# colmap/glomap

Hardware: NVIDIA H100
Metric: observations/sec per BA LM-iteration (higher is better)
Workload: dtype f64

## Files before the change

glomap_b200/csrc/ba_kernels_ext.cuh:

```cuda
#pragma once
#include "ba_kernels_v3.cuh"

namespace b200 {

struct ExtView {
  int C, K, S;
  const IntrVarRec* ivar;
  const unsigned char* sensor_var;
};

template <bool WK, bool WS>
struct ObsFull {
  double Jr[6], Jt[6], Jp[6], r[2], rho0;
  double Jk[WK ? 2 : 1][kMaxBlockDof];
  double Jsr[WS ? 6 : 1], Jst[WS ? 6 : 1];
  bool valid;
};

template <bool WK, bool WS>
__device__ __forceinline__ void obs_full(const double4& q4, const double4& t4, const double* __restrict__ ir,
                                         const IntrVarRec& iv, const double* __restrict__ sr, bool svar, double X0,
                                         double X1, double X2, double2 xy, double huber_a, ObsFull<WK, WS>& o) {
  const int mask = (int)(__double_as_longlong(t4.w) & 0xff);
  const double q[4] = {q4.x, q4.y, q4.z, q4.w};
// ... 120 lines not shown
  const double4 q4c = ld_rec32(cam_rec + (size_t)cam * kCamRec);
  const double4 t4c = ld_rec32(cam_rec + (size_t)cam * kCamRec + 4);
  const int blk = v.seg_intr[warp];
  const double* irc = intr_rec + (size_t)blk * kIntrRec;
  const double* src = sensor_of_seg(v, warp);
  const int sidx = v.S > 0 ? v.seg_sensor[warp] : 0;
  const bool svar = v.S > 0 && ex.sensor_var && ex.sensor_var[sidx];
  IntrVarRec iv{};
  if (WHAT == 1) iv = ex.ivar[blk];
  int target = cam;
  if (WHAT == 1) {
    if (iv.mb == 0) return;
    target = ex.C + blk;
  }
  if (WHAT == 2) {
    if (!svar) return;
    target = ex.C + ex.K + sidx;
  }
  double U[21], g[6];
#pragma unroll
  for (int k = 0; k < 21; ++k) U[k] = 0.0;
#pragma unroll
  for (int k = 0; k < 6; ++k) g[k] = 0.0;
  for (int i = b + lane; i < e; i += 32) {
    const int pt = v.pt_c[i];
    const double2 xy = v.xy_c[i];
    const double X0 = points[3 * (size_t)pt], X1 = points[3 * (size_t)pt + 1], X2 = points[3 * (size_t)pt + 2];
    ObsFull<WHAT == 1, WHAT == 2> o;
    obs_full<WHAT == 1, WHAT == 2>(q4c, t4c, irc, iv, src, svar, X0, X1, X2, xy, huber_a, o);
    double Jb[2][6];
#pragma unroll
    for (int a = 0; a < 2; ++a)
#pragma unroll
      for (int k = 0; k < 3; ++k) {
        if (WHAT == 0) { Jb[a][k] = o.Jr[3 * a + k]; Jb[a][3 + k] = o.Jt[3 * a + k]; }
        if (WHAT == 2) { Jb[a][k] = o.Jsr[WHAT == 2 ? 3 * a + k : 0]; Jb[a][3 + k] = o.Jst[WHAT == 2 ? 3 * a + k : 0]; }
      }
    if (WHAT == 1) {
#pragma unroll
      for (int a = 0; a < 2; ++a) {
#pragma unroll
        for (int j = 0; j < kMaxBlockDof; ++j) Jb[a][j] = o.Jk[WHAT == 1 ? a : 0][j];
        Jb[a][5] = 0.0;
      }
    }
    int idx = 0;
#pragma unroll
    for (int i2 = 0; i2 < 6; ++i2) {
#pragma unroll
      for (int j = i2; j < 6; ++j) U[idx++] += Jb[0][i2] * Jb[0][j] + Jb[1][i2] * Jb[1][j];
      g[i2] += Jb[0][i2] * o.r[0] + Jb[1][i2] * o.r[1];
    }
  }
#pragma unroll
  for (int k = 0; k < 21; ++k) {
    const double s = warp_sum(U[k]);
    if (lane == k && s != 0.0) atomicAdd(&v.U[(size_t)target * 21 + k], s);
  }
#pragma unroll
  for (int k = 0; k < 6; ++k) {
    const double s = warp_sum(g[k]);
    if (lane == 21 + k && s != 0.0) atomicAdd(&v.gc[(size_t)target * 6 + k], s);
  }
}

template <int MODE, bool WK, bool WS>
__global__ void __launch_bounds__(kEllThreads) bax_pass_a(BAView v, EllView ell, ExtView ex, BAViewV2 v2,
                                                           const double* __restrict__ cam_rec,
                                                           const double* __restrict__ intr_rec,
                                                           const double* __restrict__ x, const double* __restrict__ points,
                                                           double* __restrict__ points_new, double huber_a, double radius,
                                                           double* __restrict__ bscal, const PcgCtl* __restrict__ ctl) {
  __shared__ double scratch[32];
  if (ctl && ctl->done) return;
  const int slot = blockIdx.x * kEllThreads + threadIdx.x;
  const int lane = threadIdx.x & 31;
  const int g = slot >> 5;
  double b0 = 0, b1 = 0, b2 = 0, b3 = 0;
  if (g < ell.n_groups) {
    const int pt = ell.pt[slot];
    const int mylen = ell.len[slot];
    const int r0 = ell.row0[g], nrow = ell.row0[g + 1] - r0;
    double X0 = 0, X1 = 0, X2 = 0;
    if (pt >= 0) {
      X0 = points[3 * (size_t)pt]; X1 = points[3 * (size_t)pt + 1]; X2 = points[3 * (size_t)pt + 2];
    }
    double s0 = 0, s1 = 0, s2 = 0;
    for (int j = 0; j < nrow; ++j) {
      if (j >= mylen) continue;
      const size_t idx = ((size_t)r0 + j) * 32 + lane;
      const int cam = ell.cam[idx];
      const double2 xy = ell.xy[idx];
      const double4 q4 = ld_rec32(cam_rec + (size_t)cam * kCamRec);
      const double4 t4 = ld_rec32(cam_rec + (size_t)cam * kCamRec + 4);
      const int sidx = ell.sensor ? (int)ell.sensor[idx] : 0;
      const double* sr = ell.sensor ? v.sensor_rec + (size_t)sidx * kSensorRec : nullptr;
      const int blk = obs_intr_idx(t4, sr);
      const double* ir = intr_rec + (size_t)blk * kIntrRec;
      const bool svar = WS && ell.sensor && ex.sensor_var && ex.sensor_var[sidx];
      IntrVarRec iv{};
      if (WK) iv = ex.ivar[blk];
      ObsFull<WK, WS> o;
      obs_full<WK, WS>(q4, t4, ir, iv, sr, svar, X0, X1, X2, xy, huber_a, o);
      double xc[6], xk[kMaxBlockDof], xs[6];
#pragma unroll
      for (int k = 0; k < 6; ++k) xc[k] = x[(size_t)cam * 6 + k];
#pragma unroll
      for (int k = 0; k < kMaxBlockDof; ++k) xk[k] = WK ? x[(size_t)(ex.C + blk) * 6 + k] : 0.0;
#pragma unroll
      for (int k = 0; k < 6; ++k) xs[k] = (WS && svar) ? x[(size_t)(ex.C + ex.K + sidx) * 6 + k] : 0.0;
      double t0, t1;
      obs_apply<WK, WS>(o, xc, xk, xs, t0, t1);
      s0 += o.Jp[0] * t0 + o.Jp[3] * t1;
      s1 += o.Jp[1] * t0 + o.Jp[4] * t1;
      s2 += o.Jp[2] * t0 + o.Jp[5] * t1;
    }
// ... 53 lines not shown
                                                 const double* __restrict__ x, double huber_a, double* __restrict__ y,
                                                 const PcgCtl* __restrict__ ctl) {
  if (ctl && ctl->done) return;
  const int warp = (blockIdx.x * blockDim.x + threadIdx.x) >> 5;
  const int lane = threadIdx.x & 31;
  if (warp >= v.n_segs) return;
  const int cam = v.seg_cam[warp];
  const int b = v.seg_begin[warp], e = v.seg_end[warp];
  const double4 q4c = ld_rec32(cam_rec + (size_t)cam * kCamRec);
  const double4 t4c = ld_rec32(cam_rec + (size_t)cam * kCamRec + 4);
  const int blk = v.seg_intr[warp];
  const double* irc = intr_rec + (size_t)blk * kIntrRec;
  const double* src = sensor_of_seg(v, warp);
  const int sidx = v.S > 0 ? v.seg_sensor[warp] : 0;
  const bool svar = WS && v.S > 0 && ex.sensor_var && ex.sensor_var[sidx];
  IntrVarRec iv{};
  if (WK) iv = ex.ivar[blk];
  double xc[6], xk[kMaxBlockDof], xs[6];
#pragma unroll
  for (int k = 0; k < 6; ++k) xc[k] = x ? x[(size_t)cam * 6 + k] : 0.0;
#pragma unroll
  for (int k = 0; k < kMaxBlockDof; ++k) xk[k] = (WK && x) ? x[(size_t)(ex.C + blk) * 6 + k] : 0.0;
#pragma unroll
  for (int k = 0; k < 6; ++k) xs[k] = (WS && svar && x) ? x[(size_t)(ex.C + ex.K + sidx) * 6 + k] : 0.0;
  double ac[6] = {0, 0, 0, 0, 0, 0}, ak[kMaxBlockDof] = {0, 0, 0, 0, 0}, as[6] = {0, 0, 0, 0, 0, 0};
  for (int i = b + lane; i < e; i += 32) {
    const int pt = v.pt_c[i];
    const double2 xy = v.xy_c[i];
    const double X0 = points[3 * (size_t)pt], X1 = points[3 * (size_t)pt + 1], X2 = points[3 * (size_t)pt + 2];
    const double4 z = *reinterpret_cast<const double4*>(v2.z4 + 4 * (size_t)pt);
    ObsFull<WK, WS> o;
    obs_full<WK, WS>(q4c, t4c, irc, iv, src, svar, X0, X1, X2, xy, huber_a, o);
    double t0, t1;
    obs_apply<WK, WS>(o, xc, xk, xs, t0, t1);
    t0 -= o.Jp[0] * z.x + o.Jp[1] * z.y + o.Jp[2] * z.z;
    t1 -= o.Jp[3] * z.x + o.Jp[4] * z.y + o.Jp[5] * z.z;
#pragma unroll
    for (int k = 0; k < 3; ++k) {
      ac[k] += o.Jr[k] * t0 + o.Jr[3 + k] * t1;
      ac[3 + k] += o.Jt[k] * t0 + o.Jt[3 + k] * t1;
    }
    if (WK) {
#pragma unroll
      for (int j = 0; j < kMaxBlockDof; ++j) ak[j] += o.Jk[0][j] * t0 + o.Jk[WK ? 1 : 0][j] * t1;
    }
    if (WS) {
#pragma unroll
      for (int k = 0; k < 3; ++k) {
        as[k] += o.Jsr[WS ? k : 0] * t0 + o.Jsr[WS ? 3 + k : 0] * t1;
        as[3 + k] += o.Jst[WS ? k : 0] * t0 + o.Jst[WS ? 3 + k : 0] * t1;
      }
    }
  }
#pragma unroll
  for (int k = 0; k < 6; ++k) {
    const double s = warp_sum(ac[k]);
    if (lane == k && s != 0.0) atomicAdd(&y[(size_t)cam * 6 + k], s);
  }
  if (WK) {
#pragma unroll
    for (int j = 0; j < kMaxBlockDof; ++j) {
      const double s = warp_sum(ak[j]);
      if (lane == 8 + j && j < iv.mb && s != 0.0) atomicAdd(&y[(size_t)(ex.C + blk) * 6 + j], s);
    }
  }
  if (WS) {
#pragma unroll
    for (int k = 0; k < 6; ++k) {
      const double s = warp_sum(as[k]);
      if (lane == 16 + k && svar && s != 0.0) atomicAdd(&y[(size_t)(ex.C + ex.K + sidx) * 6 + k], s);
    }
  }
}

__global__ void bax_update_extras(ExtView ex, const IntrVarRec* __restrict__ ivar, const int* __restrict__ intr_model,
                                  const double* __restrict__ intr, double* __restrict__ intr_new,
                                  const double* __restrict__ sq, const double* __restrict__ st, double* __restrict__ sq_new,
                                  double* __restrict__ st_new, const double* __restrict__ dc, const double* __restrict__ gc,
                                  const double* __restrict__ resid, const double* __restrict__ Dc,
                                  const double* __restrict__ jscale_c, const double* __restrict__ blk_used, int count_norms,
                                  double* __restrict__ cscal) {
  const int i = blockIdx.x * blockDim.x + threadIdx.x;
  double a0 = 0, a1 = 0, a2 = 0, a3 = 0, a4 = 0;
  if (i < ex.K) {
    const IntrVarRec iv = ivar[i];
    const size_t blk = (size_t)(ex.C + i);
    double p[12];
#pragma unroll
    for (int j = 0; j < 12; ++j) p[j] = intr[(size_t)i * 12 + j];
    for (int j = 0; j < iv.mb; ++j) {
      const size_t k = blk * 6 + j;
      if (!(jscale_c[k] >= 0.0)) continue;
      const double d = dc[k];
      a0 += gc[k] * d;
      a1 += resid[k] * d;
      a2 += Dc[k] * d * d;
      a3 += d * d;
      p[iv.pidx[j]] += d;
    }
    if (iv.mb > 0 && blk_used[blk] > 0.0) {
      const int npar = intr_model[i] == 0 ? 3 : (intr_model[i] == 3 ? 5 : 4);
      for (int j = 0; j < npar; ++j) a4 += intr[(size_t)i * 12 + j] * intr[(size_t)i * 12 + j];
    }
#pragma unroll
    for (int j = 0; j < 12; ++j) intr_new[(size_t)i * 12 + j] = p[j];
  } else if (i < ex.K + ex.S) {
    const int s = i - ex.K;
    const size_t blk = (size_t)(ex.C + ex.K + s);
    double d[6];
    bool rvar = false, tvar = false;
#pragma unroll
    for (int k = 0; k < 6; ++k) {
      const size_t j = blk * 6 + k;
      const bool var = jscale_c[j] >= 0.0;
      d[k] = var ? dc[j] : 0.0;
      if (var) {
        a0 += gc[j] * d[k];
        a1 += resid[j] * d[k];
        a2 += Dc[j] * d[k] * d[k];
        if (k < 3) rvar = true; else tvar = true;
      }
    }
    const bool in_problem = ex.sensor_var && ex.sensor_var[s] && blk_used[blk] > 0.0;
    const double q[4] = {sq[4 * s], sq[4 * s + 1], sq[4 * s + 2], sq[4 * s + 3]};
    double qn[4] = {q[0], q[1], q[2], q[3]};
// ... 43 lines not shown
```

glomap_b200/csrc/ba_kernels_v2.cuh:

```cuda
#pragma once
#include "ba_kernels.cuh"
#include "pcg.cuh"

namespace b200 {

struct BAViewV2 {
  const double* Ap;
  double* z4;
  const double* pts4;
  double* Ufk = nullptr;
  const IntrVarRec* ivar = nullptr;
  int C = 0;
};

template <int NK>
__device__ __forceinline__ void obs_intr_jac(const ObsCore& o, const Intr& in, const IntrVarRec& iv,
                                             double Jk[2][NK > 0 ? NK : 1]) {
#pragma unroll
  for (int j = 0; j < NK; ++j) {
    double jx = 0.0, jy = 0.0;
    if (j < iv.mb) intr_param_jac(in, iv.pidx[j], o.uv[0], o.uv[1], 1.0, jx, jy);
    if (!o.valid) jx = jy = 0.0;
    Jk[0][j] = jx;
    Jk[1][j] = jy;
  }
}
template <int NK>
__device__ __forceinline__ void obs_intr_rows(const ObsCore& o, const Intr& in, const IntrVarRec& iv,
                                              const double Jp[6], double Jk[2][NK > 0 ? NK : 1],
                                              double B[NK > 0 ? 3 * NK : 1]) {
  obs_intr_jac<NK>(o, in, iv, Jk);
#pragma unroll
  for (int j = 0; j < NK; ++j)
#pragma unroll
    for (int c = 0; c < 3; ++c) B[3 * j + c] = o.rho1 * (Jp[c] * Jk[0][j] + Jp[3 + c] * Jk[1][j]);
}

struct SegRec {
  double R[9];
  double4 t4;
  Intr in;
  const double* sr;
};
__device__ __forceinline__ void seg_records(const BAView& v, int seg, int cam, const double* __restrict__ cam_rec,
                                            const double* __restrict__ intr_rec, SegRec& s) {
  const double4 q4 = ld_rec32(cam_rec + (size_t)cam * kCamRec);
  s.t4 = ld_rec32(cam_rec + (size_t)cam * kCamRec + 4);
  s.in = ld_intr(intr_rec + (size_t)v.seg_intr[seg] * kIntrRec);
  s.sr = sensor_of_seg(v, seg);
  const double q[4] = {q4.x, q4.y, q4.z, q4.w};
  quat_to_R(q, s.R);
}
__device__ __forceinline__ void to_sensor(const double* __restrict__ sr, double x[3]) {
  if (!sr) return;
  const double x0 = x[0], x1 = x[1], x2 = x[2];
#pragma unroll
  for (int k = 0; k < 3; ++k) x[k] = sr[3 * k] * x0 + sr[3 * k + 1] * x1 + sr[3 * k + 2] * x2;
}
__device__ __forceinline__ void cam_frame_jac(const ObsCore& o, const double r[3], double a[2], double w[3]) {
  const ProjJac& p = o.pj;
  const double t0 = r[0] - p.u * r[2], t1 = r[1] - p.v * r[2];
  const double c = o.rho1 * p.iz;
  a[0] = c * (p.m00 * t0 + p.m01 * t1);
  a[1] = c * (p.m10 * t0 + p.m11 * t1);
  const double s0 = p.iz * (p.m00 * a[0] + p.m10 * a[1]), s1 = p.iz * (p.m01 * a[0] + p.m11 * a[1]);
  w[0] = s0;
  w[1] = s1;
  w[2] = -(p.u * s0 + p.v * s1);
}
__device__ __forceinline__ void rig_to_frame(const double* __restrict__ sr, double x[3]) {
  const double x0 = x[0], x1 = x[1], x2 = x[2];
#pragma unroll
  for (int k = 0; k < 3; ++k) x[k] = sr[k] * x0 + sr[3 + k] * x1 + sr[6 + k] * x2;
}

constexpr int kXqStride = 8;
__global__ void ba2_pack_x(int C, const double* __restrict__ x, const double* __restrict__ cam_rec,
                           double* __restrict__ xp) {
  const int c = blockIdx.x * blockDim.x + threadIdx.x;
  if (c >= C) return;
  const double* r = cam_rec + (size_t)c * kCamRec;
  const double q[4] = {r[0], r[1], r[2], r[3]};
  double R[9];
  quat_to_R(q, R);
  const double* xc = x + (size_t)c * 6;
  double* o = xp + (size_t)c * kXqStride;
#pragma unroll
  for (int k = 0; k < 3; ++k) {
    o[k] = R[k] * xc[0] + R[3 + k] * xc[1] + R[6 + k] * xc[2];
    o[3 + k] = R[k] * xc[3] + R[3 + k] * xc[4] + R[6 + k] * xc[5];
  }
}

__global__ void __launch_bounds__(kPcgThreads) ba2_pcg_direction_pack(int nb, int nblk, int it, int min_it, double rel_tol,
                                                                      const double* __restrict__ z, double* __restrict__ p,
                                                                      double* __restrict__ yw,
                                                                      const double* __restrict__ dots_pp,
                                                                      const double* __restrict__ part_rz,
                                                                      const double* __restrict__ part_rr,
                                                                      double* __restrict__ dots_pub, PcgCtl* __restrict__ ctl,
                                                                      const double* __restrict__ cam_rec,
                                                                      double* __restrict__ xp, int n_pack) {
  __shared__ double sh3[3];
  double beta;
  if (!pcg_direction_head(nblk, it, min_it, rel_tol, dots_pp, part_rz, part_rr, nullptr, dots_pub, ctl, sh3, beta)) return;
  const int c = blockIdx.x * blockDim.x + threadIdx.x;
  if (c >= nb) return;
  double pv[6];
#pragma unroll
  for (int k = 0; k < 6; ++k) {
    const size_t i = (size_t)c * 6 + k;
    pv[k] = (it == 1) ? z[i] : z[i] + beta * p[i];
    p[i] = pv[k];
    yw[i] = 0.0;
  }
  if (c >= n_pack) return;
  const double* r = cam_rec + (size_t)c * kCamRec;
  const double q[4] = {r[0], r[1], r[2], r[3]};
  double R[9];
  quat_to_R(q, R);
  double* o = xp + (size_t)c * kXqStride;
#pragma unroll
  for (int k = 0; k < 3; ++k) {
    o[k] = R[k] * pv[0] + R[3 + k] * pv[1] + R[6 + k] * pv[2];
    o[3 + k] = R[k] * pv[3] + R[3 + k] * pv[4] + R[6 + k] * pv[5];
  }
// ... 46 lines not shown
    if (i + 32 < e) pt_nxt = ld_stream(v.pt_c + i + 32);
    xy = ld_stream(v.xy_c + i);
    Xc = ld_rec32(pts4 + 4 * (size_t)pt0);
  }
  for (; i < e; i += 32) {
    double4 Xn = Xc;
    double2 xyn = xy;
    int pt_nn = 0;
    if (i + 32 < e) {
      Xn = ld_rec32(pts4 + 4 * (size_t)pt_nxt);
      xyn = ld_stream(v.xy_c + i + 32);
    }
    if (i + 64 < e) pt_nn = ld_stream(v.pt_c + i + 64);
    const double X0 = Xc.x, X1 = Xc.y, X2 = Xc.z;
    ObsCore o;
    obs_core_R(sg.R, sg.t4, sg.in, sg.sr, X0, X1, X2, xy, huber_a, o);
    double Jc[2][6];
#pragma unroll
    for (int a = 0; a < 2; ++a) {
      const double j0 = o.J[3 * a], j1 = o.J[3 * a + 1], j2 = o.J[3 * a + 2];
      Jc[a][0] = rvar ? -2.0 * (j1 * o.RX[2] - j2 * o.RX[1]) : 0.0;
      Jc[a][1] = rvar ? -2.0 * (j2 * o.RX[0] - j0 * o.RX[2]) : 0.0;
      Jc[a][2] = rvar ? -2.0 * (j0 * o.RX[1] - j1 * o.RX[0]) : 0.0;
      Jc[a][3] = tvar ? j0 : 0.0;
      Jc[a][4] = tvar ? j1 : 0.0;
      Jc[a][5] = tvar ? j2 : 0.0;
    }
    const double e0 = o.rho1 * o.e[0], e1 = o.rho1 * o.e[1];
    int idx = 0;
#pragma unroll
    for (int i2 = 0; i2 < 6; ++i2) {
      const double s0 = o.rho1 * Jc[0][i2], s1 = o.rho1 * Jc[1][i2];
#pragma unroll
      for (int j = i2; j < 6; ++j) U[idx++] += s0 * Jc[0][j] + s1 * Jc[1][j];
      g[i2] += Jc[0][i2] * e0 + Jc[1][i2] * e1;
    }
    if (NK > 0) {
      double Jk[2][NKK];
      obs_intr_jac<NK>(o, sg.in, iv, Jk);
      int ik = 0;
#pragma unroll
      for (int a = 0; a < NK; ++a) {
        const double s0 = o.rho1 * Jk[0][a], s1 = o.rho1 * Jk[1][a];
#pragma unroll
        for (int c = a; c < NK; ++c) Ukk[ik++] += s0 * Jk[0][c] + s1 * Jk[1][c];
        gk[a] += Jk[0][a] * e0 + Jk[1][a] * e1;
#pragma unroll
        for (int i2 = 0; i2 < 6; ++i2) Ufk[i2][a] += Jc[0][i2] * s0 + Jc[1][i2] * s1;
      }
    }
    Xc = Xn; xy = xyn; pt_nxt = pt_nn;
  }
  if (NK > 0) {
    const size_t kb = (size_t)(v2.C + blk);
    int ik = 0;
#pragma unroll
    for (int a = 0; a < NK; ++a) {
#pragma unroll
      for (int c = a; c < NK; ++c) {
        const double sacc = warp_sum(Ukk[ik++]);
        if (lane == 0 && sacc != 0.0) atomicAdd(&v.U[kb * 21 + sym_idx(6, a, c)], sacc);
      }
      const double sg = warp_sum(gk[a]);
      if (lane == 0 && sg != 0.0) atomicAdd(&v.gc[kb * 6 + a], sg);
#pragma unroll
      for (int i2 = 0; i2 < 6; ++i2) {
        const double sf = warp_sum(Ufk[i2][a]);
        if (lane == 0 && sf != 0.0) atomicAdd(&v2.Ufk[((size_t)cam * 6 + i2) * NK + a], sf);
      }
    }
  }
#pragma unroll
  for (int k = 0; k < 21; ++k) {
    const double s = warp_sum(U[k]);
    if (lane == k && s != 0.0) atomicAdd(&v.U[(size_t)cam * 21 + k], s);
  }
#pragma unroll
  for (int k = 0; k < 6; ++k) {
    const double s = warp_sum(g[k]);
    if (lane == 21 + k && s != 0.0) atomicAdd(&v.gc[(size_t)cam * 6 + k], s);
  }
}

__global__ void __launch_bounds__(128, B200_SD_MIN_CTAS) ba2_schur_diag(BAView v, BAViewV2 v2, const double* __restrict__ cam_rec,
                                                                        const double* __restrict__ intr_rec, double huber_a) {
  const int warp = (blockIdx.x * blockDim.x + threadIdx.x) >> 5;
  const int lane = threadIdx.x & 31;
  if (warp >= v.n_segs) return;
  const int cam = v.seg_cam[warp];
  const int b = v.seg_begin[warp], e = v.seg_end[warp];
  SegRec sg;
  seg_records(v, warp, cam, cam_rec, intr_rec, sg);
  double RR[6] = {0, 0, 0, 0, 0, 0}, RT[9] = {0, 0, 0, 0, 0, 0, 0, 0, 0}, TT[6] = {0, 0, 0, 0, 0, 0};
  int i = b + lane;
  int pt_nxt = 0;
  double2 xy = make_double2(0, 0), va = xy, vb = xy, vc = xy;
  double4 Xc = make_double4(0, 0, 0, 0);
  if (i < e) {
    const int pt0 = ld_stream(v.pt_c + i);
    if (i + 32 < e) pt_nxt = ld_stream(v.pt_c + i + 32);
    xy = ld_stream(v.xy_c + i);
    Xc = ld_rec32(v2.pts4 + 4 * (size_t)pt0);
    const double2* vp = reinterpret_cast<const double2*>(v.Vinv + (size_t)pt0 * 6);
    va = vp[0]; vb = vp[1]; vc = vp[2];
  }
  for (; i < e; i += 32) {
    double4 Xn = Xc;
    double2 xyn = xy, van = va, vbn = vb, vcn = vc;
    int pt_nn = 0;
    if (i + 32 < e) {
      Xn = ld_rec32(v2.pts4 + 4 * (size_t)pt_nxt);
      xyn = ld_stream(v.xy_c + i + 32);
      const double2* vp = reinterpret_cast<const double2*>(v.Vinv + (size_t)pt_nxt * 6);
      van = vp[0]; vbn = vp[1]; vcn = vp[2];
    }
    if (i + 64 < e) pt_nn = ld_stream(v.pt_c + i + 64);
    ObsCore o;
    obs_core_R(sg.R, sg.t4, sg.in, sg.sr, Xc.x, Xc.y, Xc.z, xy, huber_a, o);
    double X[3] = {o.RX[0], o.RX[1], o.RX[2]};
    to_sensor(sg.sr, X);
    const ProjJac& pj = o.pj;
    const double vi[6] = {va.x, va.y, vb.x, vb.y, vc.x, vc.y};
    double e0[3] = {1.0, 0.0, -pj.u}, e1[3] = {0.0, 1.0, -pj.v};
    if (sg.sr) {
#pragma unroll
      for (int c = 0; c < 3; ++c) {
        e0[c] = sg.sr[c] - pj.u * sg.sr[6 + c];
        e1[c] = sg.sr[3 + c] - pj.v * sg.sr[6 + c];
      }
    }
    double l0[3], l1[3], t0[3], t1[3];
#pragma unroll
    for (int c = 0; c < 3; ++c) {
      l0[c] = e0[0] * sg.R[c] + e0[1] * sg.R[3 + c] + e0[2] * sg.R[6 + c];
      l1[c] = e1[0] * sg.R[c] + e1[1] * sg.R[3 + c] + e1[2] * sg.R[6 + c];
    }
    sym3_mul(vi, l0, t0);
    sym3_mul(vi, l1, t1);
    const double q00 = l0[0] * t0[0] + l0[1] * t0[1] + l0[2] * t0[2];
    const double q01 = l0[0] * t1[0] + l0[1] * t1[1] + l0[2] * t1[2];
    const double q11 = l1[0] * t1[0] + l1[1] * t1[1] + l1[2] * t1[2];
    const double k00 = pj.m00 * pj.m00 + pj.m10 * pj.m10, k01 = pj.m00 * pj.m01 + pj.m10 * pj.m11,
                 k11 = pj.m01 * pj.m01 + pj.m11 * pj.m11;
    const double a00 = k00 * q00 + k01 * q01, a01 = k00 * q01 + k01 * q11;
    const double a10 = k01 * q00 + k11 * q01, a11 = k01 * q01 + k11 * q11;
    const double sc = o.rho1 * pj.iz * pj.iz, c2 = sc * sc;
    const double h00 = c2 * (a00 * k00 + a01 * k01), h01 = c2 * (a00 * k01 + a01 * k11), h11 = c2 * (a10 * k01 + a11 * k11);
    double N[3][3];
    N[0][0] = h00; N[0][1] = N[1][0] = h01; N[1][1] = h11;
    N[0][2] = N[2][0] = -(h00 * pj.u + h01 * pj.v);
    N[1][2] = N[2][1] = -(h01 * pj.u + h11 * pj.v);
    N[2][2] = -(N[0][2] * pj.u + N[1][2] * pj.v);
    double P[3][3];
#pragma unroll
    for (int c = 0; c < 3; ++c) {
      const double n0 = N[0][c], n1 = N[1][c], n2 = N[2][c];
      P[0][c] = 2.0 * (X[1] * n2 - X[2] * n1);
      P[1][c] = 2.0 * (X[2] * n0 - X[0] * n2);
      P[2][c] = 2.0 * (X[0] * n1 - X[1] * n0);
    }
    double PK[3][3];
#pragma unroll
    for (int r = 0; r < 3; ++r) {
      PK[r][0] = P[r][1] * X[2] - P[r][2] * X[1];
      PK[r][1] = -P[r][0] * X[2] + P[r][2] * X[0];
      PK[r][2] = P[r][0] * X[1] - P[r][1] * X[0];
    }
    RR[0] += -2.0 * PK[0][0]; RR[1] += -2.0 * PK[0][1]; RR[2] += -2.0 * PK[0][2];
    RR[3] += -2.0 * PK[1][1]; RR[4] += -2.0 * PK[1][2]; RR[5] += -2.0 * PK[2][2];
#pragma unroll
    for (int r = 0; r < 3; ++r)
#pragma unroll
      for (int c = 0; c < 3; ++c) RT[3 * r + c] += P[r][c];
    TT[0] += N[0][0]; TT[1] += N[0][1]; TT[2] += N[0][2]; TT[3] += N[1][1]; TT[4] += N[1][2]; TT[5] += N[2][2];
    Xc = Xn; xy = xyn; va = van; vb = vbn; vc = vcn; pt_nxt = pt_nn;
  }
#pragma unroll
  for (int k = 0; k < 6; ++k) RR[k] = warp_sum(RR[k]);
#pragma unroll
  for (int k = 0; k < 9; ++k) RT[k] = warp_sum(RT[k]);
#pragma unroll
  for (int k = 0; k < 6; ++k) TT[k] = warp_sum(TT[k]);
  if (lane == 0) {
    const int mask = (int)(__double_as_longlong(sg.t4.w) & 0xff);
    double R[9] = {1, 0, 0, 0, 1, 0, 0, 0, 1};
    if (sg.sr) {
      for (int r = 0; r < 3; ++r)
        for (int c = 0; c < 3; ++c) R[3 * r + c] = sg.sr[3 * c + r];
    }
    double M[6][6];
    const double rr[3][3] = {{RR[0], RR[1], RR[2]}, {RR[1], RR[3], RR[4]}, {RR[2], RR[4], RR[5]}};
    const double tt[3][3] = {{TT[0], TT[1], TT[2]}, {TT[1], TT[3], TT[4]}, {TT[2], TT[4], TT[5]}};
    for (int r = 0; r < 3; ++r)
      for (int c = 0; c < 3; ++c) {
        M[r][c] = rr[r][c];
        M[3 + r][3 + c] = tt[r][c];
        M[r][3 + c] = RT[3 * r + c];
        M[3 + c][r] = RT[3 * r + c];
      }
    double T[6][6];
    for (int blk = 0; blk < 2; ++blk)
      for (int r = 0; r < 3; ++r)
        for (int c = 0; c < 6; ++c)
          T[3 * blk + r][c] = R[3 * r] * M[3 * blk][c] + R[3 * r + 1] * M[3 * blk + 1][c] + R[3 * r + 2] * M[3 * blk + 2][c];
    int idx = 0;
    for (int r = 0; r < 6; ++r)
      for (int c = r; c < 6; ++c, ++idx) {
        const int cb = c / 3, cc = c % 3;
        double s = T[r][3 * cb] * R[3 * cc] + T[r][3 * cb + 1] * R[3 * cc + 1] + T[r][3 * cb + 2] * R[3 * cc + 2];
        const bool rfix = (r < 3) ? (mask & 1) : (mask & 2), cfix = (c < 3) ? (mask & 1) : (mask & 2);
        if (rfix || cfix) s = 0.0;
        if (s != 0.0) atomicAdd(&v.Sd[(size_t)cam * 21 + idx], s);
      }
  }
}

struct K3v2Smem {
  alignas(128) double At[kTile * kJpDoubles];
  double t[3][kTile + 1];
  double z[3][kTilePts + 1];
  double X[3][kTilePts + 1];
  unsigned pb[kTilePts + 1];
  double scratch[32];
  alignas(8) uint64_t mbar;
};

template <int MODE>
__global__ void __launch_bounds__(kTile, MODE == 0 ? B200_PA_MIN_CTAS : B200_K3_MIN_CTAS) ba2_pass_a(BAView v, BAViewV2 v2, const double* __restrict__ xp,
                                                                     const double* __restrict__ points,
                                                                     double* __restrict__ points_new, double radius,
                                                                     double* __restrict__ bscal,
                                                                     const PcgCtl* __restrict__ ctl) {
  extern __shared__ __align__(128) unsigned char smem_raw[];
  if (ctl && ctl->done) return;
  K3v2Smem& sm = *reinterpret_cast<K3v2Smem*>(smem_raw);
  const int tile = blockIdx.x;
  const int tid = threadIdx.x;
  const int4 td = v.tile_desc[tile];
  const int p0 = td.x, npts = td.y, n = td.w;
  const unsigned o0 = (unsigned)td.z, o1 = o0 + (unsigned)n;
  const int nchunks = (n + kTile - 1) / kTile;
  constexpr uint32_t kRowBytes = kJpDoubles * 8;
  if (tid == 0) {
    mbar_init(&sm.mbar, 1);
    fence_mbar_init();
    if (n > 0) {
      const int nc0 = min(kTile, n);
      mbar_arrive_expect_tx(&sm.mbar, (uint32_t)nc0 * kRowBytes);
      tma_load_1d_stream(sm.At, v2.Ap + (size_t)o0 * kJpDoubles, (uint32_t)nc0 * kRowBytes, &sm.mbar);
    }
  }
  double xr0 = 0, xr1 = 0, xr2 = 0, xt0 = 0;
  double2 xt12 = make_double2(0, 0);
  int pl_pf = 0;
  if (tid < n) {
    const int cam = ld_stream(v.obs_cam + o0 + tid);
    pl_pf = ld_stream(v.obs_pt + o0 + tid) - p0;
    ld_nc_256(xp + (size_t)cam * kXqStride, xr0, xr1, xr2, xt0);
    xt12 = __ldg(reinterpret_cast<const double2*>(xp + (size_t)cam * kXqStride + 4));
  }
  if (tid < npts) {
    sm.pb[tid] = v.pt_begin[p0 + tid];
    if (tid == npts - 1) sm.pb[npts] = o1;
#pragma unroll
    for (int k = 0; k < 3; ++k) sm.X[k][tid] = points[3 * (size_t)(p0 + tid) + k];
    sm.z[0][tid] = sm.z[1][tid] = sm.z[2][tid] = 0.0;
  }
// ... 149 lines not shown
  constexpr int NKK = NK > 0 ? NK : 1;
  IntrVarRec iv{};
  if (NK > 0) iv = v2.ivar[blk];
  double acc[6] = {0, 0, 0, 0, 0, 0};
  double accK[NKK];
#pragma unroll
  for (int k = 0; k < NKK; ++k) accK[k] = 0.0;
  const uint64_t keep = l2_policy_evict_last();
  int i = b + lane;
  int pt_nxt = 0;
  double4 X = make_double4(0, 0, 0, 0), z = X;
  double2 xy = make_double2(0, 0);
  if (i < e) {
    const int pt0 = ld_stream(v.pt_c + i);
    if (i + 32 < e) pt_nxt = ld_stream(v.pt_c + i + 32);
    X = ld_rec32(v2.pts4 + 4 * (size_t)pt0);
    z = ld_keep4(v2.z4 + 4 * (size_t)pt0, keep);
    xy = ld_stream(v.xy_c + i);
  }
  for (; i < e; i += 32) {
    double4 Xn = X, zn = z;
    double2 xyn = xy;
    int pt_nn = 0;
    if (i + 32 < e) {
      Xn = ld_rec32(v2.pts4 + 4 * (size_t)pt_nxt);
      zn = ld_keep4(v2.z4 + 4 * (size_t)pt_nxt, keep);
      xyn = ld_stream(v.xy_c + i + 32);
    }
    if (i + 64 < e) pt_nn = ld_stream(v.pt_c + i + 64);
    ObsCore o;
    obs_core_R(sg.R, sg.t4, sg.in, sg.sr, X.x, X.y, X.z, xy, huber_a, o);
    double P[3] = {o.RX[0], o.RX[1], o.RX[2]};
    to_sensor(sg.sr, P);
    double r[3] = {sg.R[0] * z.x + sg.R[1] * z.y + sg.R[2] * z.z,
                   sg.R[3] * z.x + sg.R[4] * z.y + sg.R[5] * z.z,
                   sg.R[6] * z.x + sg.R[7] * z.y + sg.R[8] * z.z};
    to_sensor(sg.sr, r);
    double a[2], w[3];
    cam_frame_jac(o, r, a, w);
    acc[0] += P[1] * w[2] - P[2] * w[1];
    acc[1] += P[2] * w[0] - P[0] * w[2];
    acc[2] += P[0] * w[1] - P[1] * w[0];
    acc[3] += w[0];
    acc[4] += w[1];
    acc[5] += w[2];
    if (NK > 0) {
      double Jk[2][NKK];
      obs_intr_jac<NK>(o, sg.in, iv, Jk);
#pragma unroll
      for (int k = 0; k < NK; ++k) accK[k] += Jk[0][k] * a[0] + Jk[1][k] * a[1];
    }
    X = Xn; z = zn; xy = xyn; pt_nxt = pt_nn;
  }
#pragma unroll
  for (int k = 0; k < 6; ++k) acc[k] = warp_sum(acc[k]);
  if (sg.sr) {
    rig_to_frame(sg.sr, acc);
    rig_to_frame(sg.sr, acc + 3);
  }
  const int mask = (int)(__double_as_longlong(sg.t4.w) & 0xff);
#pragma unroll
  for (int k = 0; k < 6; ++k) {
    const double s = k < 3 ? 2.0 * acc[k] : acc[k];
    const bool fixed = k < 3 ? (mask & 1) : (mask & 2);
    if (lane == k && !fixed && s != 0.0) atomicAdd(&y[(size_t)cam * 6 + k], -s);
  }
  if (NK > 0) {
    const size_t kb = (size_t)(v2.C + blk);
#pragma unroll
    for (int k = 0; k < NK; ++k) {
      const double sk = warp_sum(accK[k]);
      if (lane == 0 && sk != 0.0) atomicAdd(&y[kb * 6 + k], -sk);
    }
  }
}

__global__ void ba2k_pack_xk(int C, const double* __restrict__ cam_rec, const double* __restrict__ x, double* __restrict__ xp,
                             const PcgCtl* __restrict__ ctl) {
  if (ctl && ctl->done) return;
  const int c = blockIdx.x * blockDim.x + threadIdx.x;
  if (c >= C) return;
  const int blk = (int)(__double_as_longlong(cam_rec[(size_t)c * kCamRec + 7]) >> 8);
  xp[(size_t)c * kXqStride + 6] = x[(size_t)(C + blk) * 6];
  xp[(size_t)c * kXqStride + 7] = x[(size_t)(C + blk) * 6 + 1];
}

template <int NK>
__global__ void __launch_bounds__(256) ba2k_cross(int C, int K, const double* __restrict__ cam_rec, const double* __restrict__ Ufk,
                                                  const double* __restrict__ x, double* __restrict__ y,
                                                  const PcgCtl* __restrict__ ctl) {
  constexpr int kBins = 256;
  __shared__ double bins[kBins * NK];
  if (ctl && ctl->done) return;
  const bool use_bins = K <= kBins;
  if (use_bins) {
    for (int i = threadIdx.x; i < K * NK; i += blockDim.x) bins[i] = 0.0;
    __syncthreads();
  }
  const int c = blockIdx.x * blockDim.x + threadIdx.x;
  if (c < C) {
    const int blk = (int)(__double_as_longlong(cam_rec[(size_t)c * kCamRec + 7]) >> 8);
    double xf[6], xk[NK], tk[NK];
#pragma unroll
    for (int i = 0; i < 6; ++i) xf[i] = x[(size_t)c * 6 + i];
#pragma unroll
    for (int k = 0; k < NK; ++k) {
      xk[k] = x[(size_t)(C + blk) * 6 + k];
      tk[k] = 0.0;
    }
    const double* u = Ufk + (size_t)c * 6 * NK;
#pragma unroll
    for (int i = 0; i < 6; ++i) {
      double yf = 0.0;
#pragma unroll
      for (int k = 0; k < NK; ++k) {
        const double uik = u[i * NK + k];
        yf += uik * xk[k];
        tk[k] += uik * xf[i];
      }
      if (yf != 0.0) y[(size_t)c * 6 + i] += yf;
    }
#pragma unroll
    for (int k = 0; k < NK; ++k) {
      if (tk[k] == 0.0) continue;
      if (use_bins) atomicAdd(&bins[blk * NK + k], tk[k]);
      else atomicAdd(&y[(size_t)(C + blk) * 6 + k], tk[k]);
// ... 11 lines not shown
```

glomap_b200/csrc/common.cuh:

```cuda
#pragma once
#include <cuda_runtime.h>
#include <stdint.h>
#include <stdio.h>

#include <string>

namespace b200 {

#ifndef B200_TILE
#define B200_TILE 128
#endif
#ifndef B200_K1_MIN_CTAS
#define B200_K1_MIN_CTAS 5
#endif
#ifndef B200_K3_MIN_CTAS
#define B200_K3_MIN_CTAS 8
#endif
#ifndef B200_PA_MIN_CTAS
#define B200_PA_MIN_CTAS 12
#endif
#ifndef B200_LC_MIN_CTAS
#define B200_LC_MIN_CTAS 3
#endif
#ifndef B200_PB_MIN_CTAS
// ... 115 lines not shown
  return __ldcs(p);
#else
  return *p;
#endif
}
template <class T>
__device__ __forceinline__ void st_stream(T* p, T v) {
#if B200_STREAM_HINTS
  __stcs(p, v);
#else
  *p = v;
#endif
}
#ifndef B200_KEEP_HINTS
#define B200_KEEP_HINTS 0
#endif
__device__ __forceinline__ uint64_t l2_policy_evict_last() {
  uint64_t p;
  asm volatile("createpolicy.fractional.L2::evict_last.b64 %0, 1.0;" : "=l"(p));
  return p;
}
__device__ __forceinline__ double4 ld_keep4(const double* p, uint64_t pol) {
#if B200_KEEP_HINTS
  double4 v;
  asm volatile("ld.global.L2::cache_hint.v2.f64 {%0, %1}, [%2], %3;" : "=d"(v.x), "=d"(v.y) : "l"(p), "l"(pol));
  asm volatile("ld.global.L2::cache_hint.v2.f64 {%0, %1}, [%2], %3;" : "=d"(v.z), "=d"(v.w) : "l"(p + 2), "l"(pol));
  return v;
#else
  return ld_rec32(p);
#endif
}
__device__ __forceinline__ void st_keep4(double* p, double4 v, uint64_t pol) {
#if B200_KEEP_HINTS
  asm volatile("st.global.L2::cache_hint.v2.f64 [%0], {%1, %2}, %3;" ::"l"(p), "d"(v.x), "d"(v.y), "l"(pol) : "memory");
  asm volatile("st.global.L2::cache_hint.v2.f64 [%0], {%1, %2}, %3;" ::"l"(p + 2), "d"(v.z), "d"(v.w), "l"(pol) : "memory");
#else
  st_rec32(p, v.x, v.y, v.z, v.w);
#endif
}
__device__ __forceinline__ void tma_store_1d(void* gdst, const void* smem_src, uint32_t bytes) {
  asm volatile("cp.async.bulk.global.shared::cta.bulk_group [%0], [%1], %2;" ::"l"(gdst), "r"(smem_u32(smem_src)),
               "r"(bytes)
               : "memory");
}
__device__ __forceinline__ void tma_store_commit() { asm volatile("cp.async.bulk.commit_group;" ::: "memory"); }
__device__ __forceinline__ void tma_store_wait_read() { asm volatile("cp.async.bulk.wait_group.read 0;" ::: "memory"); }
__device__ __forceinline__ void tma_store_wait_all() { asm volatile("cp.async.bulk.wait_group 0;" ::: "memory"); }

__device__ __forceinline__ double warp_sum(double v) {
#pragma unroll
  for (int o = 16; o > 0; o >>= 1) v += __shfl_xor_sync(0xffffffffu, v, o);
  return v;
}
__device__ __forceinline__ double warp_max(double v) {
#pragma unroll
  for (int o = 16; o > 0; o >>= 1) v = fmax(v, __shfl_xor_sync(0xffffffffu, v, o));
  return v;
}
__device__ __forceinline__ double block_sum(double v, double* scratch) {
  v = warp_sum(v);
  const int lane = threadIdx.x & 31, w = threadIdx.x >> 5;
  __syncthreads();
  if (lane == 0) scratch[w] = v;
  __syncthreads();
  const int nw = (blockDim.x + 31) >> 5;
  v = (threadIdx.x < nw) ? scratch[threadIdx.x] : 0.0;
  if (w == 0) v = warp_sum(v);
  return v;
}
__device__ __forceinline__ double block_max(double v, double* scratch) {
  v = warp_max(v);
  const int lane = threadIdx.x & 31, w = threadIdx.x >> 5;
  __syncthreads();
  if (lane == 0) scratch[w] = v;
  __syncthreads();
  const int nw = (blockDim.x + 31) >> 5;
  v = (threadIdx.x < nw) ? scratch[threadIdx.x] : 0.0;
  if (w == 0) v = warp_max(v);
  return v;
}
__device__ __forceinline__ void atomic_max_nonneg(double* addr, double v) {
  atomicMax(reinterpret_cast<unsigned long long*>(addr), (unsigned long long)__double_as_longlong(v));
}

__device__ __forceinline__ bool sym3_inverse(const double a[6], double inv[6]) {
  const double c00 = a[3] * a[5] - a[4] * a[4];
  const double c01 = a[2] * a[4] - a[1] * a[5];
  const double c02 = a[1] * a[4] - a[2] * a[3];
  const double det = a[0] * c00 + a[1] * c01 + a[2] * c02;
  if (!(fabs(det) > 0.0)) {
    inv[0] = inv[1] = inv[2] = inv[3] = inv[4] = inv[5] = 0.0;
    return false;
  }
  const double id = 1.0 / det;
  inv[0] = c00 * id;
  inv[1] = c01 * id;
  inv[2] = c02 * id;
  inv[3] = (a[0] * a[5] - a[2] * a[2]) * id;
  inv[4] = (a[1] * a[2] - a[0] * a[4]) * id;
  inv[5] = (a[0] * a[3] - a[1] * a[1]) * id;
  return true;
}
__device__ __forceinline__ void sym3_mul(const double a[6], const double v[3], double out[3]) {
  out[0] = a[0] * v[0] + a[1] * v[1] + a[2] * v[2];
  out[1] = a[1] * v[0] + a[3] * v[1] + a[4] * v[2];
  out[2] = a[2] * v[0] + a[4] * v[1] + a[5] * v[2];
// ... 81 lines not shown
```

profiles/sass_excerpt.py:

```python
#!/usr/bin/env python
import collections
import os
import re
import subprocess

ROOT = os.path.dirname(os.path.dirname(os.path.abspath(__file__)))
KERNELS = ["ba3_linearize_points", "ba2_linearize_cams", "ba3_pass_a", "ba2_pass_b", "ba2_schur_diag", "ba3_cost",
           "ba2_pcg_direction_pack", "pcg_update", "pcg_apply_diag", "bax_pass_b", "ba2k_cross", "gp_schur_pass", "ra_laplacian_csr",
           "ra2_laplacian_dot", "ra2_coarse", "p2p_allreduce_sum", "proc_undistort", "trk_hook"]
KEEP = re.compile(r"^(LDG|STG|LDS|STS|RED|ATOM|BAR|SHFL|DFMA|DMUL|DADD|MUFU|CCTL|UBLKCP|SYNCS|MEMBAR|ERRBAR|LDGSTS)")
LOOP_KERNELS = ["ba2_pass_b", "ba2_schur_diag", "ba2_linearize_cams", "ba3_pass_a"]
FP64 = re.compile(r"^(DFMA|DMUL|DADD|DSETP|DMNMX|MUFU)")
LOADS = re.compile(r"^(LDG|LD|LDS|LDL|LDC)\b")
INSN = re.compile(r"/\*([0-9a-f]{4,})\*/\s+(?:@!?U?P\w+\s+)?([A-Z0-9_.]+)([^;]*);")


def inner_loop(insns):
    best = None
    for addr, op, args in insns:
        m = re.search(r"0x([0-9a-f]+)\s*$", args.strip())
        if op.startswith("BRA") and m and int(m.group(1), 16) < addr:
            body = [(a, o) for a, o, _ in insns if int(m.group(1), 16) <= a <= addr]
            if best is None or len(body) > len(best):
                best = body
    if not best:
        return None
    ops = [o for _, o in best]
    return len(ops), sum(bool(FP64.match(o)) for o in ops), sum(bool(LOADS.match(o)) for o in ops)


def main():
    lib = os.path.join(ROOT, "glomap_b200", "libb200sfm.so")
    txt = subprocess.run(["cuobjdump", "-sass", lib], capture_output=True, text=True).stdout
    names = subprocess.run(["cu++filt"], input="\n".join(re.findall(r"Function : (\S+)", txt)), capture_output=True, text=True).stdout.split("\n")
    mangled = re.findall(r"Function : (\S+)", txt)
    demangle = dict(zip(mangled, names))
    cur, counts, totals = None, collections.defaultdict(collections.Counter), collections.Counter()
    insns = collections.defaultdict(list)
    for line in txt.splitlines():
        m = re.search(r"Function : (\S+)", line)
        if m:
            cur = demangle.get(m.group(1), m.group(1))
            continue
        m = INSN.search(line)
        if m and cur:
            totals[cur] += 1
            op = m.group(2)
            insns[cur].append((int(m.group(1), 16), op, m.group(3)))
            if KEEP.match(op):
                counts[cur][op] += 1
    print("# SASS mnemonics of the hot kernels (cuobjdump -sass glomap_b200/libb200sfm.so, sm_90a)")
    print("# per kernel: total instructions, then the memory / synchronisation / FP64 mnemonics with their static counts")
    print("# (profiles/sass_excerpt.py regenerates this file; no tensor-core or TMA mnemonics are expected: FP64 streaming kernels)\n")
    for k in sorted(counts):
        if not any(re.search(r"\b" + re.escape(n) + r"\b", k) for n in KERNELS):
            continue
        ops = ", ".join(f"{o} x{c}" for o, c in counts[k].most_common(14))
        print(k[:200])
        print(f"    total {totals[k]} instructions: {ops}")
        if any(re.search(r"\b" + n + r"\b", k) for n in LOOP_KERNELS):
            loop = inner_loop(insns[k])
            if loop:
                print(f"    inner loop: {loop[0]} instructions, {loop[1]} FP64 + MUFU, {loop[2]} loads")


if __name__ == "__main__":
    main()
```

Before: 1.556 billion.

## Replace per-value warp_sum epilogues with a butterfly warp reduce-scatter

Adds a warp_reduce_scatter helper that reduces up to 32 per-lane values across a warp with a halving butterfly, leaving each reduced value on a distinct lane. It uses about 31 shuffles in total instead of 5 per value. The segment epilogues of the linearize, pass_b, schur_diag and extension kernels now use it, and each lane issues its own atomicAdd. The rig rotation in schur_diag and pass_b is spread across lanes through a small shared-memory stage instead of being done serially by lane 0. The aim is to cut shuffle count and serial lane-0 work in kernel tails, at the cost of more index arithmetic and register pressure.

After: 1.606 billion, median of 6. +3.2%, better.

```diff
diff --git a/glomap_b200/csrc/ba_kernels_ext.cuh b/glomap_b200/csrc/ba_kernels_ext.cuh
--- a/glomap_b200/csrc/ba_kernels_ext.cuh
+++ b/glomap_b200/csrc/ba_kernels_ext.cuh
@@ -196,16 +196,14 @@
       g[i2] += Jb[0][i2] * o.r[0] + Jb[1][i2] * o.r[1];
     }
   }
-#pragma unroll
-  for (int k = 0; k < 21; ++k) {
-    const double s = warp_sum(U[k]);
-    if (lane == k && s != 0.0) atomicAdd(&v.U[(size_t)target * 21 + k], s);
-  }
-#pragma unroll
-  for (int k = 0; k < 6; ++k) {
-    const double s = warp_sum(g[k]);
-    if (lane == 21 + k && s != 0.0) atomicAdd(&v.gc[(size_t)target * 6 + k], s);
-  }
+  double vals[27];
+#pragma unroll
+  for (int k = 0; k < 21; ++k) vals[k] = U[k];
+#pragma unroll
+  for (int k = 0; k < 6; ++k) vals[21 + k] = g[k];
+  const double s = warp_reduce_scatter(vals);
+  if (lane < 27 && s != 0.0)
+    atomicAdd(lane < 21 ? &v.U[(size_t)target * 21 + lane] : &v.gc[(size_t)target * 6 + (lane - 21)], s);
 }
 
 template <int MODE, bool WK, bool WS>
@@ -365,25 +363,26 @@
       }
     }
   }
-#pragma unroll
-  for (int k = 0; k < 6; ++k) {
-    const double s = warp_sum(ac[k]);
-    if (lane == k && s != 0.0) atomicAdd(&y[(size_t)cam * 6 + k], s);
-  }
-  if (WK) {
-#pragma unroll
-    for (int j = 0; j < kMaxBlockDof; ++j) {
-      const double s = warp_sum(ak[j]);
-      if (lane == 8 + j && j < iv.mb && s != 0.0) atomicAdd(&y[(size_t)(ex.C + blk) * 6 + j], s);
-    }
-  }
-  if (WS) {
-#pragma unroll
-    for (int k = 0; k < 6; ++k) {
-      const double s = warp_sum(as[k]);
-      if (lane == 16 + k && svar && s != 0.0) atomicAdd(&y[(size_t)(ex.C + ex.K + sidx) * 6 + k], s);
-    }
-  }
+  constexpr int NKV = WK ? kMaxBlockDof : 0, KV = 6 + NKV + (WS ? 6 : 0), S = warp_rs_stride<KV>();
+  double vals[KV];
+#pragma unroll
+  for (int k = 0; k < 6; ++k) vals[k] = ac[k];
+#pragma unroll
+  for (int j = 0; j < NKV; ++j) vals[6 + j] = ak[j];
+#pragma unroll
+  for (int k = 0; k < (WS ? 6 : 0); ++k) vals[6 + NKV + k] = as[k];
+  const double s = warp_reduce_scatter(vals);
+  const int k = lane / S;
+  bool live = lane % S == 0 && k < KV && s != 0.0;
+  double* dst = &y[(size_t)cam * 6 + k];
+  if (k >= 6 && k < 6 + NKV) {
+    live = live && k - 6 < iv.mb;
+    dst = &y[(size_t)(ex.C + blk) * 6 + (k - 6)];
+  } else if (k >= 6 + NKV) {
+    live = live && svar;
+    dst = &y[(size_t)(ex.C + ex.K + sidx) * 6 + (k - 6 - NKV)];
+  }
+  if (live) atomicAdd(dst, s);
 }
 
 __global__ void bax_update_extras(ExtView ex, const IntrVarRec* __restrict__ ivar, const int* __restrict__ intr_model,
diff --git a/glomap_b200/csrc/ba_kernels_v2.cuh b/glomap_b200/csrc/ba_kernels_v2.cuh
--- a/glomap_b200/csrc/ba_kernels_v2.cuh
+++ b/glomap_b200/csrc/ba_kernels_v2.cuh
@@ -67,11 +67,6 @@
   w[0] = s0;
   w[1] = s1;
   w[2] = -(p.u * s0 + p.v * s1);
-}
-__device__ __forceinline__ void rig_to_frame(const double* __restrict__ sr, double x[3]) {
-  const double x0 = x[0], x1 = x[1], x2 = x[2];
-#pragma unroll
-  for (int k = 0; k < 3; ++k) x[k] = sr[k] * x0 + sr[3 + k] * x1 + sr[6 + k] * x2;
 }
 
 constexpr int kXqStride = 8;
@@ -224,36 +219,55 @@
     Xc = Xn; xy = xyn; pt_nxt = pt_nn;
   }
   if (NK > 0) {
+    constexpr int nU = NKK * (NKK + 1) / 2, KV = nU + NKK + 6 * NKK, S = warp_rs_stride<KV>();
+    double vals[KV];
+#pragma unroll
+    for (int k = 0; k < nU; ++k) vals[k] = Ukk[k];
+#pragma unroll
+    for (int a = 0; a < NKK; ++a) {
+      vals[nU + a] = gk[a];
+#pragma unroll
+      for (int i2 = 0; i2 < 6; ++i2) vals[nU + NKK + i2 * NKK + a] = Ufk[i2][a];
+    }
+    const double s = warp_reduce_scatter(vals);
+    const int k = lane / S;
     const size_t kb = (size_t)(v2.C + blk);
+    double* dst = &v2.Ufk[(size_t)cam * 6 * NKK + (k - nU - NKK)];
+    if (k < nU + NKK) dst = &v.gc[kb * 6 + (k - nU)];
     int ik = 0;
 #pragma unroll
-    for (int a = 0; a < NK; ++a) {
-#pragma unroll
-      for (int c = a; c < NK; ++c) {
-        const double sacc = warp_sum(Ukk[ik++]);
-        if (lane == 0 && sacc != 0.0) atomicAdd(&v.U[kb * 21 + sym_idx(6, a, c)], sacc);
-      }
-      const double sg = warp_sum(gk[a]);
-      if (lane == 0 && sg != 0.0) atomicAdd(&v.gc[kb * 6 + a], sg);
-#pragma unroll
-      for (int i2 = 0; i2 < 6; ++i2) {
-        const double sf = warp_sum(Ufk[i2][a]);
-        if (lane == 0 && sf != 0.0) atomicAdd(&v2.Ufk[((size_t)cam * 6 + i2) * NK + a], sf);
-      }
-    }
-  }
-#pragma unroll
-  for (int k = 0; k < 21; ++k) {
-    const double s = warp_sum(U[k]);
-    if (lane == k && s != 0.0) atomicAdd(&v.U[(size_t)cam * 21 + k], s);
-  }
-#pragma unroll
-  for (int k = 0; k < 6; ++k) {
-    const double s = warp_sum(g[k]);
-    if (lane == 21 + k && s != 0.0) atomicAdd(&v.gc[(size_t)cam * 6 + k], s);
-  }
-}
-
+    for (int a = 0; a < NKK; ++a)
+#pragma unroll
+      for (int c = a; c < NKK; ++c, ++ik)
+        if (k == ik) dst = &v.U[kb * 21 + sym_idx(6, a, c)];
+    if (lane % S == 0 && k < KV && s != 0.0) atomicAdd(dst, s);
+  }
+  double vals[27];
+#pragma unroll
+  for (int k = 0; k < 21; ++k) vals[k] = U[k];
+#pragma unroll
+  for (int k = 0; k < 6; ++k) vals[21 + k] = g[k];
+  const double s = warp_reduce_scatter(vals);
+  if (lane < 27 && s != 0.0) atomicAdd(lane < 21 ? &v.U[(size_t)cam * 21 + lane] : &v.gc[(size_t)cam * 6 + (lane - 21)], s);
+}
+
+__device__ __forceinline__ void sd_entry(int k, int& r, int& c) {
+  if (k >= 6 && k < 15) {
+    r = (k - 6) / 3;
+    c = 3 + (k - 6) % 3;
+  } else {
+    const int o = k < 6 ? 0 : 3, t = k < 6 ? k : k - 15;
+    const int i = (t >= 3) + (t >= 5);
+    r = o + i;
+    c = o + t - (i == 0 ? 0 : i == 1 ? 2 : 3);
+  }
+}
+__device__ __forceinline__ int sd_value(int p, int q) {
+  const int i = min(p, q), j = max(p, q);
+  if (j < 3) return sym_idx(3, i, j);
+  if (i >= 3) return 15 + sym_idx(3, i - 3, j - 3);
+  return 6 + 3 * i + (j - 3);
+}
 __global__ void __launch_bounds__(128, B200_SD_MIN_CTAS) ba2_schur_diag(BAView v, BAViewV2 v2, const double* __restrict__ cam_rec,
                                                                         const double* __restrict__ intr_rec, double huber_a) {
   const int warp = (blockIdx.x * blockDim.x + threadIdx.x) >> 5;
@@ -347,44 +361,35 @@
     TT[0] += N[0][0]; TT[1] += N[0][1]; TT[2] += N[0][2]; TT[3] += N[1][1]; TT[4] += N[1][2]; TT[5] += N[2][2];
     Xc = Xn; xy = xyn; va = van; vb = vbn; vc = vcn; pt_nxt = pt_nn;
   }
-#pragma unroll
-  for (int k = 0; k < 6; ++k) RR[k] = warp_sum(RR[k]);
-#pragma unroll
-  for (int k = 0; k < 9; ++k) RT[k] = warp_sum(RT[k]);
-#pragma unroll
-  for (int k = 0; k < 6; ++k) TT[k] = warp_sum(TT[k]);
-  if (lane == 0) {
-    const int mask = (int)(__double_as_longlong(sg.t4.w) & 0xff);
-    double R[9] = {1, 0, 0, 0, 1, 0, 0, 0, 1};
-    if (sg.sr) {
-      for (int r = 0; r < 3; ++r)
-        for (int c = 0; c < 3; ++c) R[3 * r + c] = sg.sr[3 * c + r];
-    }
-    double M[6][6];
-    const double rr[3][3] = {{RR[0], RR[1], RR[2]}, {RR[1], RR[3], RR[4]}, {RR[2], RR[4], RR[5]}};
-    const double tt[3][3] = {{TT[0], TT[1], TT[2]}, {TT[1], TT[3], TT[4]}, {TT[2], TT[4], TT[5]}};
-    for (int r = 0; r < 3; ++r)
-      for (int c = 0; c < 3; ++c) {
-        M[r][c] = rr[r][c];
-        M[3 + r][3 + c] = tt[r][c];
-        M[r][3 + c] = RT[3 * r + c];
-        M[3 + c][r] = RT[3 * r + c];
-      }
-    double T[6][6];
-    for (int blk = 0; blk < 2; ++blk)
-      for (int r = 0; r < 3; ++r)
-        for (int c = 0; c < 6; ++c)
-          T[3 * blk + r][c] = R[3 * r] * M[3 * blk][c] + R[3 * r + 1] * M[3 * blk + 1][c] + R[3 * r + 2] * M[3 * blk + 2][c];
-    int idx = 0;
-    for (int r = 0; r < 6; ++r)
-      for (int c = r; c < 6; ++c, ++idx) {
-        const int cb = c / 3, cc = c % 3;
-        double s = T[r][3 * cb] * R[3 * cc] + T[r][3 * cb + 1] * R[3 * cc + 1] + T[r][3 * cb + 2] * R[3 * cc + 2];
-        const bool rfix = (r < 3) ? (mask & 1) : (mask & 2), cfix = (c < 3) ? (mask & 1) : (mask & 2);
-        if (rfix || cfix) s = 0.0;
-        if (s != 0.0) atomicAdd(&v.Sd[(size_t)cam * 21 + idx], s);
-      }
-  }
+  double vals[21];
+#pragma unroll
+  for (int k = 0; k < 6; ++k) vals[k] = RR[k];
+#pragma unroll
+  for (int k = 0; k < 9; ++k) vals[6 + k] = RT[k];
+#pragma unroll
+  for (int k = 0; k < 6; ++k) vals[15 + k] = TT[k];
+  double s = warp_reduce_scatter(vals);
+  int r, c;
+  sd_entry(lane, r, c);
+  if (sg.sr) {
+    __shared__ double stage[4][21];
+    double* st = stage[threadIdx.x >> 5];
+    if (lane < 21) st[lane] = s;
+    __syncwarp();
+    if (lane < 21) {
+      const int rb = r - r % 3, cb = c - c % 3;
+      const double* sr = sg.sr;
+      double t[3];
+#pragma unroll
+      for (int j = 0; j < 3; ++j)
+        t[j] = sr[r % 3] * st[sd_value(rb, cb + j)] + sr[3 + r % 3] * st[sd_value(rb + 1, cb + j)] +
+               sr[6 + r % 3] * st[sd_value(rb + 2, cb + j)];
+      s = t[0] * sr[c % 3] + t[1] * sr[3 + c % 3] + t[2] * sr[6 + c % 3];
+    }
+  }
+  const int mask = (int)(__double_as_longlong(sg.t4.w) & 0xff);
+  const bool rfix = (r < 3) ? (mask & 1) : (mask & 2), cfix = (c < 3) ? (mask & 1) : (mask & 2);
+  if (lane < 21 && !rfix && !cfix && s != 0.0) atomicAdd(&v.Sd[(size_t)cam * 21 + sym_idx(6, r, c)], s);
 }
 
 struct K3v2Smem {
@@ -640,26 +645,29 @@
     }
     X = Xn; z = zn; xy = xyn; pt_nxt = pt_nn;
   }
-#pragma unroll
-  for (int k = 0; k < 6; ++k) acc[k] = warp_sum(acc[k]);
+  constexpr int KV = 6 + NK, S = warp_rs_stride<KV>();
+  double vals[KV];
+#pragma unroll
+  for (int k = 0; k < 6; ++k) vals[k] = acc[k];
+#pragma unroll
+  for (int k = 0; k < NK; ++k) vals[6 + k] = accK[k];
+  double s = warp_reduce_scatter(vals);
+  const int k = lane / S;
   if (sg.sr) {
-    rig_to_frame(sg.sr, acc);
-    rig_to_frame(sg.sr, acc + 3);
+    __shared__ double stage[4][6];
+    double* st = stage[threadIdx.x >> 5];
+    if (lane % S == 0 && k < 6) st[k] = s;
+    __syncwarp();
+    if (k < 6) {
+      const int c = k % 3, h = k - c;
+      s = sg.sr[c] * st[h] + sg.sr[3 + c] * st[h + 1] + sg.sr[6 + c] * st[h + 2];
+    }
   }
   const int mask = (int)(__double_as_longlong(sg.t4.w) & 0xff);
-#pragma unroll
-  for (int k = 0; k < 6; ++k) {
-    const double s = k < 3 ? 2.0 * acc[k] : acc[k];
-    const bool fixed = k < 3 ? (mask & 1) : (mask & 2);
-    if (lane == k && !fixed && s != 0.0) atomicAdd(&y[(size_t)cam * 6 + k], -s);
-  }
-  if (NK > 0) {
-    const size_t kb = (size_t)(v2.C + blk);
-#pragma unroll
-    for (int k = 0; k < NK; ++k) {
-      const double sk = warp_sum(accK[k]);
-      if (lane == 0 && sk != 0.0) atomicAdd(&y[kb * 6 + k], -sk);
-    }
+  const bool fixed = k < 3 ? (mask & 1) : k < 6 ? (mask & 2) : false;
+  if (lane % S == 0 && k < KV && !fixed && s != 0.0) {
+    double* dst = k < 6 ? &y[(size_t)cam * 6 + k] : &y[(size_t)(v2.C + blk) * 6 + (k - 6)];
+    atomicAdd(dst, k < 3 ? -(2.0 * s) : -s);
   }
 }
 
diff --git a/glomap_b200/csrc/common.cuh b/glomap_b200/csrc/common.cuh
--- a/glomap_b200/csrc/common.cuh
+++ b/glomap_b200/csrc/common.cuh
@@ -191,6 +191,36 @@
   for (int o = 16; o > 0; o >>= 1) v += __shfl_xor_sync(0xffffffffu, v, o);
   return v;
 }
+template <int K>
+__host__ __device__ constexpr int warp_rs_stride() {
+  static_assert(K >= 1 && K <= 32, "warp_reduce_scatter takes 1..32 values");
+  return K <= 1 ? 32 : K <= 2 ? 16 : K <= 4 ? 8 : K <= 8 ? 4 : K <= 16 ? 2 : 1;
+}
+template <int M, int D>
+__device__ __forceinline__ double warp_rs_level(double* a, int lane) {
+  if constexpr (D == 0) {
+    return a[0];
+  } else if constexpr (M > 1) {
+    const bool hi = lane & D;
+#pragma unroll
+    for (int j = 0; j < M / 2; ++j) {
+      const double keep = hi ? a[M / 2 + j] : a[j], send = hi ? a[j] : a[M / 2 + j];
+      a[j] = keep + __shfl_xor_sync(0xffffffffu, send, D);
+    }
+    return warp_rs_level<M / 2, D / 2>(a, lane);
+  } else {
+    a[0] += __shfl_xor_sync(0xffffffffu, a[0], D);
+    return warp_rs_level<1, D / 2>(a, lane);
+  }
+}
+template <int K>
+__device__ __forceinline__ double warp_reduce_scatter(const double (&v)[K]) {
+  constexpr int Kp = 32 / warp_rs_stride<K>();
+  double a[Kp];
+#pragma unroll
+  for (int k = 0; k < Kp; ++k) a[k] = k < K ? v[k] : 0.0;
+  return warp_rs_level<Kp, 16>(a, threadIdx.x & 31);
+}
 __device__ __forceinline__ double warp_max(double v) {
 #pragma unroll
   for (int o = 16; o > 0; o >>= 1) v = fmax(v, __shfl_xor_sync(0xffffffffu, v, o));
diff --git a/profiles/sass_excerpt.py b/profiles/sass_excerpt.py
--- a/profiles/sass_excerpt.py
+++ b/profiles/sass_excerpt.py
@@ -3,6 +3,7 @@
 import os
 import re
 import subprocess
+import sys
 
 ROOT = os.path.dirname(os.path.dirname(os.path.abspath(__file__)))
 KERNELS = ["ba3_linearize_points", "ba2_linearize_cams", "ba3_pass_a", "ba2_pass_b", "ba2_schur_diag", "ba3_cost",
@@ -10,6 +11,9 @@
            "ra2_laplacian_dot", "ra2_coarse", "p2p_allreduce_sum", "proc_undistort", "trk_hook"]
 KEEP = re.compile(r"^(LDG|STG|LDS|STS|RED|ATOM|BAR|SHFL|DFMA|DMUL|DADD|MUFU|CCTL|UBLKCP|SYNCS|MEMBAR|ERRBAR|LDGSTS)")
 LOOP_KERNELS = ["ba2_pass_b", "ba2_schur_diag", "ba2_linearize_cams", "ba3_pass_a"]
+SEG_KERNELS = ["ba2_pass_b", "ba2_schur_diag", "ba2_linearize_cams", "bax_pass_b", "bax_linearize_blocks"]
+SHFL = re.compile(r"^SHFL\b")
+RED = re.compile(r"^(RED|REDG|ATOMG?)\.")
 FP64 = re.compile(r"^(DFMA|DMUL|DADD|DSETP|DMNMX|MUFU)")
 LOADS = re.compile(r"^(LDG|LD|LDS|LDL|LDC)\b")
 INSN = re.compile(r"/\*([0-9a-f]{4,})\*/\s+(?:@!?U?P\w+\s+)?([A-Z0-9_.]+)([^;]*);")
@@ -30,7 +34,7 @@
 
 
 def main():
-    lib = os.path.join(ROOT, "glomap_b200", "libb200sfm.so")
+    lib = sys.argv[1] if len(sys.argv) > 1 else os.path.join(ROOT, "glomap_b200", "libb200sfm.so")
     txt = subprocess.run(["cuobjdump", "-sass", lib], capture_output=True, text=True).stdout
     names = subprocess.run(["cu++filt"], input="\n".join(re.findall(r"Function : (\S+)", txt)), capture_output=True, text=True).stdout.split("\n")
     mangled = re.findall(r"Function : (\S+)", txt)
@@ -53,7 +57,7 @@
     print("# per kernel: total instructions, then the memory / synchronisation / FP64 mnemonics with their static counts")
     print("# (profiles/sass_excerpt.py regenerates this file; no tensor-core or TMA mnemonics are expected: FP64 streaming kernels)\n")
     for k in sorted(counts):
-        if not any(re.search(r"\b" + re.escape(n) + r"\b", k) for n in KERNELS):
+        if not any(re.search(r"\b" + re.escape(n) + r"\b", k) for n in KERNELS + SEG_KERNELS):
             continue
         ops = ", ".join(f"{o} x{c}" for o, c in counts[k].most_common(14))
         print(k[:200])
@@ -62,6 +66,11 @@
             loop = inner_loop(insns[k])
             if loop:
                 print(f"    inner loop: {loop[0]} instructions, {loop[1]} FP64 + MUFU, {loop[2]} loads")
+        if any(re.search(r"\b" + n + r"\b", k) for n in SEG_KERNELS):
+            ops = [o for _, o, _ in insns[k]]
+            red = collections.Counter(o for o in ops if RED.match(o))
+            print(f"    segment epilogue: SHFL x{sum(bool(SHFL.match(o)) for o in ops)}, global reductions "
+                  + (", ".join(f"{o} x{c}" for o, c in red.most_common()) or "none"))
 
 
 if __name__ == "__main__":
```
